# rezashkv/diffusion_pruning

Measured on NVIDIA B200. Metric: mixed_expert_unet_samples_steps_per_s, higher is better.
Workload: dtype bf16

## Files before the change

diffusion_pruning_b200/csrc/gemm_sm100.cu:

```cuda
#include "common.cuh"
#include "../../include/aptp_sm100.h"

namespace aptp {

constexpr int BM = 128;
constexpr int BK = 64;
constexpr int A_STAGE_BYTES = BM * BK * 2;
constexpr int EPI_PER_QUAD = 3;
constexpr int EPI_WARPS = 4 * EPI_PER_QUAD;
constexpr int GEMM_THREADS = 128 + EPI_WARPS * 32;
#define GEMM_CTRL_REGS "56"
#define GEMM_EPI_REGS "152"
constexpr int TMEM_COLS = 512;
constexpr int STG_WARP_BYTES = 32 * 64;
constexpr int STG_BYTES = EPI_WARPS * STG_WARP_BYTES;
constexpr int MAX_SMEM_SEGS = 96;
constexpr int SSEG_BYTES = MAX_SMEM_SEGS * 48;
constexpr int TILE_CACHE = 160;
constexpr int STILE_BYTES = TILE_CACHE * 16;
constexpr int SBIAS_BYTES = EPI_WARPS * 128 * 4;

struct GemmParams {
  CUtensorMap tmap_a;
  CUtensorMap tmap_b;
  CUtensorMap tmap_out;
  int out_tma;
  const aptp_gemm_seg* segs;
  const aptp_gemm_tile* tiles;
  int n_tiles;
  int n_segs;
  int a_mode;
  int batch, Ho, Wo;
  int bn, bw, bh, bb;
  int lbw, lbh;
  int stages;
  int k_tap_pitch;
  void* out;
  int out_ld, out_mode;
  const float* bias;
  const float* rowvec;
  int rowvec_ld, rows_per_sample;
  const void* residual;
  int res_ld;
  const float* gate;
  int gate_ld, gate_group;
  const float* border_tab;
  int tab_ld;
  int flags;
  const float* ln_colsum;
  const float2* ln_rowstats;
  float2* rowstat_out;
  int rowstat_chunks;
  float* gn_sum;
  float* gn_sq;
  int gn_ld, gn_blocks;
  int a_stat;
  int halo;
  CUtensorMap tmap_a2;
  CUtensorMap tmap_b2;
// ... 73 lines not shown
    v[q * 4 + 2] += f.z;
    v[q * 4 + 3] += f.w;
  }
}

__device__ __forceinline__ void ln_bias_apply32(float* v, const float* bias, const float* cs, float mu, float rstd) {
  const uint64_t r2 = pack_f32x2(rstd, rstd);
  const float nm = -mu * rstd;
  const uint64_t n2 = pack_f32x2(nm, nm);
#pragma unroll
  for (int q = 0; q < 8; ++q) {
    const float4 b = *(reinterpret_cast<const float4*>(bias) + q);
    const float4 c = *(reinterpret_cast<const float4*>(cs) + q);
    uint64_t a0 = fma_f32x2(r2, pack_f32x2(v[q * 4 + 0], v[q * 4 + 1]), pack_f32x2(b.x, b.y));
    uint64_t a1 = fma_f32x2(r2, pack_f32x2(v[q * 4 + 2], v[q * 4 + 3]), pack_f32x2(b.z, b.w));
    a0 = fma_f32x2(n2, pack_f32x2(c.x, c.y), a0);
    a1 = fma_f32x2(n2, pack_f32x2(c.z, c.w), a1);
    unpack_f32x2(a0, v[q * 4 + 0], v[q * 4 + 1]);
    unpack_f32x2(a1, v[q * 4 + 2], v[q * 4 + 3]);
  }
}

enum { EPI_BF16 = 0, EPI_GEGLU = 1, EPI_F32 = 2, EPI_NCHW = 3 };
#ifdef APTP_GEMM_TRACE
__device__ long long g_gemm_trace[512][16];
#define TRACE_T0() const long long _t0 = clock64(); long long _tw[2] = {0, 0}
#define TRACE_ADD(slot) if (lane == 0) { g_gemm_trace[blockIdx.x][slot] += clock64() - _t0; g_gemm_trace[blockIdx.x][slot + 1] += _tw[1]; if (slot == 2) g_gemm_trace[blockIdx.x][4] += _tw[0]; }
#define TRACE_WAIT(slot, expr) [&]() { const long long _w0 = clock64(); const bool _r = (expr); _tw[slot & 1] += clock64() - _w0; return _r; }()
#else
#define TRACE_T0()
#define TRACE_ADD(slot)
#define TRACE_WAIT(slot, expr) (expr)
#endif
template <int kEpi, bool k2Sm>
__global__ void __cluster_dims__(2, 1, 1) __launch_bounds__(GEMM_THREADS, 1)
grouped_gemm_kernel(const __grid_constant__ GemmParams p) {
  constexpr bool kGeglu = (kEpi == EPI_GEGLU);
  extern __shared__ uint8_t smem_raw[];
  uint8_t* smem = reinterpret_cast<uint8_t*>((reinterpret_cast<uintptr_t>(smem_raw) + 1023) & ~uintptr_t(1023));
  const int stages = p.stages;
  const uint32_t stage_bytes = ((p.a_stat || p.halo) ? 0u : (uint32_t)A_STAGE_BYTES) + (uint32_t)p.bn * (k2Sm ? 64u : 128u);
  const uint32_t ring_off = p.halo ? (uint32_t)p.halo * HALO_BYTES : (uint32_t)p.a_stat * A_STAGE_BYTES;
  uint8_t* stg_base = smem + ring_off + (size_t)stages * stage_bytes;
  float* sbias = reinterpret_cast<float*>(stg_base + STG_BYTES);
  aptp_gemm_seg* ssegs = reinterpret_cast<aptp_gemm_seg*>(stg_base + STG_BYTES + SBIAS_BYTES);
  aptp_gemm_tile* stiles = reinterpret_cast<aptp_gemm_tile*>(stg_base + STG_BYTES + SBIAS_BYTES + SSEG_BYTES);
  uint64_t* full_bar = reinterpret_cast<uint64_t*>(stg_base + STG_BYTES + SBIAS_BYTES + SSEG_BYTES + STILE_BYTES);
  uint64_t* empty_bar = full_bar + stages;
  uint64_t* tfull_bar = empty_bar + stages;
  uint64_t* tempty_bar = tfull_bar + 2;
  uint64_t* afull_bar = tempty_bar + 2;
  uint64_t* aempty_bar = afull_bar + A_STAT_MAX_CHUNKS;
  uint32_t* tmem_slot = reinterpret_cast<uint32_t*>(aempty_bar + A_STAT_MAX_CHUNKS);

  const int warp = __shfl_sync(0xffffffffu, (int)(threadIdx.x >> 5), 0);
  const int lane = threadIdx.x & 31;
#ifdef APTP_GEMM_TRACE
  const long long _t0_epi = clock64();
#endif
#define GEMM_ROLE_PROLOGUE()                                                                        \
  const uint32_t cta_rank = cluster_ctarank();                                                      \
  const int pair0 = blockIdx.x >> 1, pair_stride = gridDim.x >> 1, n_pairs = p.n_tiles >> 1;        \
  const aptp_gemm_seg* segs = (p.n_segs <= MAX_SMEM_SEGS) ? ssegs : p.segs;                         \
  const uint32_t tmem_base = *tmem_slot;                                                            \
  (void)cta_rank; (void)pair0; (void)pair_stride; (void)n_pairs; (void)segs; (void)tmem_base;

  if (warp == 0 && lane == 0) {
    tma_prefetch_desc(&p.tmap_a);
    tma_prefetch_desc(&p.tmap_b);
    if (p.out_tma) tma_prefetch_desc(&p.tmap_out);
    if (p.k2_chunks) {
      tma_prefetch_desc(&p.tmap_a2);
      tma_prefetch_desc(&p.tmap_b2);
    }
  }
  if (warp == 1) {
    if (lane == 0) {
      for (int s = 0; s < stages; ++s) {
        mbar_init(&full_bar[s], 1);
        mbar_init(&empty_bar[s], k2Sm ? 1 : 2);
      }
      for (int a = 0; a < 2; ++a) {
        mbar_init(&tfull_bar[a], 1);
        mbar_init(&tempty_bar[a], k2Sm ? 2 * EPI_WARPS : EPI_WARPS);
      }
      for (int a = 0; a < A_STAT_MAX_CHUNKS; ++a) {
        mbar_init(&afull_bar[a], 1);
        mbar_init(&aempty_bar[a], 1);
      }
      fence_barrier_init();
    }
    __syncwarp();
    if constexpr (k2Sm) {
      tmem_alloc_2sm(tmem_slot, TMEM_COLS);
      tmem_relinquish_2sm();
    } else {
      tmem_alloc(tmem_slot, TMEM_COLS);
      tmem_relinquish();
    }
  }
  const bool segs_in_smem = p.n_segs <= MAX_SMEM_SEGS;
  if (segs_in_smem) {
    const int4* src = reinterpret_cast<const int4*>(p.segs);
    int4* dst = reinterpret_cast<int4*>(ssegs);
    for (int i = threadIdx.x; i < p.n_segs * 3; i += blockDim.x) dst[i] = __ldg(src + i);
  }
  {
    const int pair0_ = blockIdx.x >> 1, pair_stride_ = gridDim.x >> 1, n_pairs_ = p.n_tiles >> 1;
    const uint32_t rank_ = cluster_ctarank();
    const int4* src = reinterpret_cast<const int4*>(p.tiles);
    int4* dst = reinterpret_cast<int4*>(stiles);
    for (int i = threadIdx.x; i < TILE_CACHE; i += blockDim.x) {
      const int pr = pair0_ + i * pair_stride_;
      if (pr < n_pairs_) dst[i] = __ldg(src + 2 * pr + rank_);
    }
  }
  tc_fence_before();
  cluster_sync_all();
  tc_fence_after();
  pdl_launch();
  pdl_wait();

// ... 295 lines not shown
            for (int k = 0; k < BK / 16; ++k) {
              if constexpr (k2Sm)
                umma_bf16_ss_2sm(d_tmem, da + (uint64_t)(k * 2), db + (uint64_t)(k * 2), idesc, (kb | k) != 0 ? 1u : 0u);
              else
                umma_bf16_ss(d_tmem, da + (uint64_t)(k * 2), db + (uint64_t)(k * 2), idesc, (kb | k) != 0 ? 1u : 0u);
            }
            if constexpr (k2Sm) umma_commit_2sm(&empty_bar[stage], (uint16_t)0x3);
            else umma_commit_mc(&empty_bar[stage], (uint16_t)0x3);
          }
          __syncwarp();
          advance(stage, phase, stages);
        }
        if (!ok) break;
        if (elect_one()) {
          if constexpr (k2Sm) umma_commit_2sm(&tfull_bar[acc], (uint16_t)0x3);
          else umma_commit(&tfull_bar[acc]);
        }
        __syncwarp();
        acc ^= 1;
        if (acc == 0) acc_phase ^= 1;
      }
      TRACE_ADD(2);
    }
  }
  } else {
    asm volatile("setmaxnreg.inc.sync.aligned.u32 " GEMM_EPI_REGS ";");
    GEMM_ROLE_PROLOGUE();
    const int ew = warp - 4;
    const int quad = warp & 3;
    const int cpar = ew >> 2;
    float* wbias = sbias + ew * 128;
    uint32_t chunk_rot = 0;
    const int r_own = quad * 32 + lane;
    uint8_t* stg = stg_base + ew * STG_WARP_BYTES;
    const uint32_t stg_own = smem_u32(stg) + lane * 64;
    const int own_sw = (lane >> 1) & 3;
    const int co_q = lane & 3;
    int acc = 0;
    uint32_t acc_phase = 0;
    constexpr bool geglu = kGeglu;
    constexpr bool bf16_out = (kEpi == EPI_BF16 || kEpi == EPI_GEGLU);
    int ti = 0;
    bool st_pending = false;
#ifdef APTP_GEMM_TRACE
    long long _tr_ld = 0, _tr_math = 0, _tr_st = 0, _tr_tfull = 0, _tr_busy = 0, _tr_tiles = 0;
#endif
    for (int pr = pair0; pr < n_pairs; pr += pair_stride, ++ti) {
      const aptp_gemm_tile tile = (ti < TILE_CACHE) ? stiles[ti] : p.tiles[2 * pr + cta_rank];
      if (tile.flags & APTP_TILE_SKIP) continue;
      const aptp_gemm_seg seg = segs[tile.seg];
      const bool placeholder = (tile.flags & APTP_TILE_PLACEHOLDER) != 0;
      TileGeom g;
      g.linear = (p.a_mode == APTP_A_LINEAR);
      g.m_base = tile.m_base;
      g.img0 = g.oy0 = g.ox0 = 0;
      if (!g.linear) {
        const int hw = p.Ho * p.Wo;
        g.img0 = tile.m_base / hw;
        const int rem = tile.m_base - g.img0 * hw;
        g.oy0 = rem / p.Wo;
        g.ox0 = rem - g.oy0 * p.Wo;
      }
      bool valid;
      int oy, ox;
      const int row = map_row(p, g, r_own, valid, oy, ox);
      valid = valid && !placeholder && (row < seg.row_end) && (row >= seg.row_begin);
      const int sample = valid ? row / p.rows_per_sample : 0;
      const int ycls = g.linear ? 1 : ((oy == 0) ? 0 : ((oy == p.Ho - 1) ? 2 : 1));
      const int xcls = g.linear ? 1 : ((ox == 0) ? 0 : ((ox == p.Wo - 1) ? 2 : 1));
      const float* tabp =
          (!kGeglu && p.border_tab) ? p.border_tab + seg.tab_off + (size_t)(ycls * 3 + xcls) * p.tab_ld : nullptr;
      int co_row[4];
      bool co_ok[4];
#pragma unroll
      for (int it = 0; it < 4; ++it) {
        int a, b;
        bool v;
        const int rr = map_row(p, g, quad * 32 + it * 8 + (lane >> 2), v, a, b);
        co_ok[it] = v && !placeholder && (rr < seg.row_end) && (rr >= seg.row_begin);
        co_row[it] = rr;
      }
      const int ocol_base = geglu ? tile.n0 / 2 : tile.n0;
      const int row0_q = tile.m_base + quad * 32;
      const bool rows_full = bf16_out && p.out_tma && !placeholder && row0_q >= seg.row_begin && row0_q + 32 <= seg.row_end;
      long long gn_row = -1;
      if ((kEpi == EPI_F32 || kEpi == EPI_BF16) && p.gn_sum != nullptr && !placeholder) {
        const int smp = tile.m_base / p.rows_per_sample;
        const int rem = tile.m_base - smp * p.rows_per_sample;
        int t_in_s;
        if (g.linear) {
          t_in_s = rem >> 7;
        } else {
          const int oy0 = rem / p.Wo, ox0 = rem - oy0 * p.Wo;
          t_in_s = (oy0 >> p.lbh) * (p.Wo >> p.lbw) + (ox0 >> p.lbw);
        }
        gn_row = ((long long)smp * p.gn_blocks + t_in_s * 4 + quad) * p.gn_ld;
      }

      uint4 rres[kEpi == EPI_BF16 ? 4 : 1];
      const bool use_res = (kEpi == EPI_BF16) && (p.residual != nullptr);
      auto load_res = [&](int col0) {
        if constexpr (kEpi == EPI_BF16) {
#pragma unroll
          for (int it = 0; it < 4; ++it) {
            rres[it] = make_uint4(0u, 0u, 0u, 0u);
            if (co_ok[it] && col0 + co_q * 8 < seg.n_valid)
              rres[it] = *reinterpret_cast<const uint4*>(reinterpret_cast<const __nv_bfloat16*>(p.residual) +
                                                         (size_t)co_row[it] * p.res_ld + seg.out_col_off + col0 +
                                                         co_q * 8);
          }
        }
      };
      constexpr bool f32_rows = (kEpi == EPI_F32);
      const bool use_res32 = f32_rows && (p.residual != nullptr) && (p.flags & APTP_EPI_RES_F32) != 0;
      uint4 rres32[f32_rows ? 2 : 1][f32_rows ? 4 : 1];
      auto load_res32 = [&](int col0) {
        if constexpr (f32_rows) {
#pragma unroll
          for (int h = 0; h < 2; ++h)
#pragma unroll
            for (int it = 0; it < 4; ++it) {
              rres32[h][it] = make_uint4(0u, 0u, 0u, 0u);
              if (co_ok[it] && col0 + h * 16 + co_q * 4 < seg.n_valid)
                rres32[h][it] = *reinterpret_cast<const uint4*>(reinterpret_cast<const float*>(p.residual) +
                                                                (size_t)co_row[it] * p.res_ld + seg.out_col_off + col0 +
                                                                h * 16 + co_q * 4);
            }
        }
      };
      const int w32_tile = (tile.flags >> 8) & 0xFF;
      const int out_cols_per_tile = geglu ? p.bn / 2 : (w32_tile ? w32_tile * 32 : p.bn);
      const int n_chunks = (out_cols_per_tile + 31) >> 5;
      const int c_first = (cpar + EPI_PER_QUAD - (int)(chunk_rot % EPI_PER_QUAD)) % EPI_PER_QUAD;
      chunk_rot += (uint32_t)n_chunks;
      const bool ln_fold = (p.flags & APTP_EPI_LN_FOLD) != 0;
      float bias_h = 0.f, bias_g = 0.f, cs_h = 0.f, cs_g = 0.f;
      auto load_bias = [&](int c) {
        const int col0 = ocol_base + c * 32;
        bias_h = bias_g = cs_h = cs_g = 0.f;
        if (p.bias && col0 + lane < seg.n_valid) {
          if (geglu) {
            bias_h = __ldg(p.bias + seg.vec_off + tile.n0 + c * 32 + lane);
            bias_g = __ldg(p.bias + seg.vec_off + tile.n0 + p.bn / 2 + c * 32 + lane);
          } else {
            bias_h = __ldg(p.bias + seg.vec_off + col0 + lane);
          }
        }
        if (ln_fold && col0 + lane < seg.n_valid) {
          if (geglu) {
            cs_h = __ldg(p.ln_colsum + seg.vec_off + tile.n0 + c * 32 + lane);
            cs_g = __ldg(p.ln_colsum + seg.vec_off + tile.n0 + p.bn / 2 + c * 32 + lane);
          } else {
            cs_h = __ldg(p.ln_colsum + seg.vec_off + col0 + lane);
          }
        }
      };
      float ln_mu = 0.f, ln_rstd = 1.f;
      if (ln_fold && valid) {
        const float2 ms = __ldg(p.ln_rowstats + row);
        ln_mu = ms.x;
        ln_rstd = ms.y;
      }
      if (c_first < n_chunks) {
        if (use_res && ocol_base + c_first * 32 < seg.n_store) load_res(ocol_base + c_first * 32);
        if (use_res32 && ocol_base + c_first * 32 < seg.n_store) load_res32(ocol_base + c_first * 32);
        load_bias(c_first);
      }

#ifdef APTP_GEMM_TRACE
      const long long _e0 = clock64();
      const bool got = mbar_wait(&tfull_bar[acc], acc_phase, p.abort_flag);
      const long long _e1 = clock64();
      _tr_tfull += _e1 - _e0;
#else
      const bool got = mbar_wait(&tfull_bar[acc], acc_phase, p.abort_flag);
#endif
      if (!got) break;
      tc_fence_after();
      asm volatile("" : "+f"(ln_mu), "+f"(ln_rstd));
      bool released = false;
      auto release_acc = [&]() {
        tc_fence_before();
        __syncwarp();
        if (lane == 0) {
          if constexpr (k2Sm) mbar_arrive_rank(&tempty_bar[acc], 0u);
          else mbar_arrive(&tempty_bar[acc]);
        }
      };
      const uint32_t t_addr = tmem_base + ((uint32_t)(quad * 32) << 16) + (uint32_t)(acc * p.bn);

#ifdef APTP_DBG_NOEPI
      if (p.n_tiles < 0)
#endif
      for (int c = c_first; c < n_chunks; c += EPI_PER_QUAD) {
        const int col0 = ocol_base + c * 32;
        if (col0 >= seg.n_store) break;
        const int n_ok = seg.n_valid - col0;
        if (st_pending) {
// ... 76 lines not shown
            release_acc();
            released = true;
          }
#endif
#pragma unroll
          for (int j = 0; j < 32; ++j) v[j] = __uint_as_float(ra[j]);
          if (ln_fold) ln_bias_apply32(v, wbias, wbias + 64, ln_mu, ln_rstd);
          else if (p.bias) add32_smem(v, wbias);
          if (p.bias || ln_fold) {
            __syncwarp();
            if (more) load_bias(c + EPI_PER_QUAD);
          }
          if (p.rowvec && valid) add32(v, p.rowvec + (size_t)sample * p.rowvec_ld + col0, n_ok);
          if (tabp) add32(v, tabp + col0, n_ok);
          if (p.gate && valid) {
            const float* gp = p.gate + (size_t)sample * p.gate_ld;
#pragma unroll
            for (int j = 0; j < 32; ++j)
              if (j < n_ok) v[j] *= __ldg(gp + (col0 + j) / p.gate_group);
          }
          if (p.flags & APTP_EPI_SILU) {
#pragma unroll
            for (int j = 0; j < 32; ++j) v[j] = silu_f(v[j]);
          }
        }

#ifdef APTP_GEMM_TRACE
        const long long _c2 = clock64();
        _tr_math += _c2 - _c1;
#endif
        if constexpr (bf16_out) {
          uint4* stg4 = reinterpret_cast<uint4*>(stg);
          if (kEpi == EPI_BF16 && use_res) {
#pragma unroll
            for (int it = 0; it < 4; ++it) {
              const int rl = it * 8 + (lane >> 2);
              stg4[rl * 4 + (co_q ^ ((rl >> 1) & 3))] = rres[it];
            }
            __syncwarp();
            uint4 w4[4];
#pragma unroll
            for (int q = 0; q < 4; ++q) w4[q] = stg4[lane * 4 + (q ^ own_sw)];
#pragma unroll
            for (int q = 0; q < 4; ++q) {
              v[q * 8 + 0] += bf16_lo(w4[q].x);
              v[q * 8 + 1] += bf16_hi(w4[q].x);
              v[q * 8 + 2] += bf16_lo(w4[q].y);
              v[q * 8 + 3] += bf16_hi(w4[q].y);
              v[q * 8 + 4] += bf16_lo(w4[q].z);
              v[q * 8 + 5] += bf16_hi(w4[q].z);
              v[q * 8 + 6] += bf16_lo(w4[q].w);
              v[q * 8 + 7] += bf16_hi(w4[q].w);
            }
            __syncwarp();
            if (more) load_res(col0 + 32 * EPI_PER_QUAD);
          }
          if (n_ok < 32) {
#pragma unroll
            for (int j = 0; j < 32; ++j)
              if (j >= n_ok) v[j] = 0.f;
          }
          if (kEpi == EPI_BF16 && p.rowstat_out && valid) {
            uint64_t su2 = pack_f32x2(0.f, 0.f), sq2 = su2;
#pragma unroll
            for (int j = 0; j < 32; j += 2) {
              const uint64_t x2 = pack_f32x2(v[j], v[j + 1]);
              su2 = add_f32x2(su2, x2);
              sq2 = fma_f32x2(x2, x2, sq2);
            }
            float s0, s1, q0, q1;
            unpack_f32x2(su2, s0, s1);
            unpack_f32x2(sq2, q0, q1);
            p.rowstat_out[(size_t)row * p.rowstat_chunks + ((seg.out_col_off + col0) >> 5)] =
                make_float2(s0 + s1, q0 + q1);
          }
#ifdef APTP_DBG_NOSTAGE
          if (v[0] == 1.2345e30f) p.abort_flag[1] = 1;
          if (p.n_tiles >= 0) continue;
#endif
#pragma unroll
          for (int q = 0; q < 4; ++q)
            stg4[lane * 4 + (q ^ own_sw)] =
                make_uint4(pack_bf16(v[q * 8 + 0], v[q * 8 + 1]), pack_bf16(v[q * 8 + 2], v[q * 8 + 3]),
                           pack_bf16(v[q * 8 + 4], v[q * 8 + 5]), pack_bf16(v[q * 8 + 6], v[q * 8 + 7]));
          if (rows_full && col0 + 32 <= seg.n_store) {
            fence_proxy_async();
            __syncwarp();
            if (lane == 0) {
              tma_store_2d(&p.tmap_out, stg, seg.out_col_off + col0, row0_q);
              bulk_commit();
            }
            st_pending = true;
            continue;
          }
          __syncwarp();
          __nv_bfloat16* obase = reinterpret_cast<__nv_bfloat16*>(p.out) + seg.out_col_off + col0 + co_q * 8;
          const bool col_ok = col0 + co_q * 8 < seg.n_store;
          uint4 o4[4];
#pragma unroll
          for (int it = 0; it < 4; ++it) {
            const int rl = it * 8 + (lane >> 2);
            o4[it] = stg4[rl * 4 + (co_q ^ ((rl >> 1) & 3))];
          }
#ifdef APTP_DBG_NOSTORE
          if (o4[0].x == 0x12345678u && o4[1].y == 0x9abcdef0u && o4[2].z == 0x0fedcba9u && o4[3].w == 0x87654321u)
#endif
#pragma unroll
          for (int it = 0; it < 4; ++it)
            if (co_ok[it] && col_ok) *reinterpret_cast<uint4*>(obase + (size_t)co_row[it] * p.out_ld) = o4[it];
          if constexpr (kEpi == EPI_BF16) {
            if (gn_row >= 0) {
              float cs[8], cq[8];
#pragma unroll
              for (int e = 0; e < 8; ++e) cs[e] = cq[e] = 0.f;
#pragma unroll
              for (int it = 0; it < 4; ++it) {
                if (co_ok[it]) {
                  const uint32_t wds[4] = {o4[it].x, o4[it].y, o4[it].z, o4[it].w};
#pragma unroll
                  for (int e = 0; e < 4; ++e) {
                    const float f0 = bf16_lo(wds[e]), f1 = bf16_hi(wds[e]);
                    cs[2 * e] += f0;
                    cs[2 * e + 1] += f1;
                    cq[2 * e] = fmaf(f0, f0, cq[2 * e]);
                    cq[2 * e + 1] = fmaf(f1, f1, cq[2 * e + 1]);
                  }
                }
              }
#pragma unroll
              for (int o = 4; o < 32; o <<= 1) {
#pragma unroll
                for (int e = 0; e < 8; ++e) {
                  cs[e] += __shfl_xor_sync(0xffffffffu, cs[e], o);
                  cq[e] += __shfl_xor_sync(0xffffffffu, cq[e], o);
                }
              }
              if (lane < 4 && col_ok) {
                const long long gi = gn_row + seg.out_col_off + col0 + co_q * 8;
                *reinterpret_cast<float4*>(p.gn_sum + gi) = make_float4(cs[0], cs[1], cs[2], cs[3]);
                *reinterpret_cast<float4*>(p.gn_sum + gi + 4) = make_float4(cs[4], cs[5], cs[6], cs[7]);
                *reinterpret_cast<float4*>(p.gn_sq + gi) = make_float4(cq[0], cq[1], cq[2], cq[3]);
                *reinterpret_cast<float4*>(p.gn_sq + gi + 4) = make_float4(cq[4], cq[5], cq[6], cq[7]);
              }
            }
          }
          __syncwarp();
        } else if constexpr (f32_rows) {
          uint4* stg4 = reinterpret_cast<uint4*>(stg);
          if (n_ok < 32) {
#pragma unroll
            for (int j = 0; j < 32; ++j)
              if (j >= n_ok) v[j] = 0.f;
          }
#pragma unroll
          for (int h = 0; h < 2; ++h) {
#pragma unroll
            for (int q = 0; q < 4; ++q)
              stg4[lane * 4 + (q ^ own_sw)] =
                  make_uint4(__float_as_uint(v[h * 16 + q * 4 + 0]), __float_as_uint(v[h * 16 + q * 4 + 1]),
                             __float_as_uint(v[h * 16 + q * 4 + 2]), __float_as_uint(v[h * 16 + q * 4 + 3]));
            __syncwarp();
            float* obase = reinterpret_cast<float*>(p.out) + seg.out_col_off + col0 + h * 16 + co_q * 4;
            const bool col_ok = col0 + h * 16 + co_q * 4 < seg.n_store;
            uint4 o4[4];
#pragma unroll
            for (int it = 0; it < 4; ++it) {
              const int rl = it * 8 + (lane >> 2);
              o4[it] = stg4[rl * 4 + (co_q ^ ((rl >> 1) & 3))];
            }
            if (use_res32) {
#pragma unroll
              for (int it = 0; it < 4; ++it) {
                o4[it].x = __float_as_uint(__uint_as_float(o4[it].x) + __uint_as_float(rres32[h][it].x));
                o4[it].y = __float_as_uint(__uint_as_float(o4[it].y) + __uint_as_float(rres32[h][it].y));
                o4[it].z = __float_as_uint(__uint_as_float(o4[it].z) + __uint_as_float(rres32[h][it].z));
                o4[it].w = __float_as_uint(__uint_as_float(o4[it].w) + __uint_as_float(rres32[h][it].w));
              }
            }
#pragma unroll
            for (int it = 0; it < 4; ++it)
              if (co_ok[it] && col_ok) *reinterpret_cast<uint4*>(obase + (size_t)co_row[it] * p.out_ld) = o4[it];
            if (gn_row >= 0) {
              float cs[4] = {0.f, 0.f, 0.f, 0.f}, cq[4] = {0.f, 0.f, 0.f, 0.f};
#pragma unroll
              for (int it = 0; it < 4; ++it) {
                if (co_ok[it]) {
                  const float f0 = __uint_as_float(o4[it].x), f1 = __uint_as_float(o4[it].y);
                  const float f2 = __uint_as_float(o4[it].z), f3 = __uint_as_float(o4[it].w);
                  cs[0] += f0; cs[1] += f1; cs[2] += f2; cs[3] += f3;
                  cq[0] = fmaf(f0, f0, cq[0]); cq[1] = fmaf(f1, f1, cq[1]);
                  cq[2] = fmaf(f2, f2, cq[2]); cq[3] = fmaf(f3, f3, cq[3]);
                }
              }
#pragma unroll
              for (int o = 4; o < 32; o <<= 1) {
#pragma unroll
                for (int e = 0; e < 4; ++e) {
                  cs[e] += __shfl_xor_sync(0xffffffffu, cs[e], o);
                  cq[e] += __shfl_xor_sync(0xffffffffu, cq[e], o);
                }
              }
              if (lane < 4 && col_ok) {
                const long long gi = gn_row + seg.out_col_off + col0 + h * 16 + co_q * 4;
                *reinterpret_cast<float4*>(p.gn_sum + gi) = make_float4(cs[0], cs[1], cs[2], cs[3]);
                *reinterpret_cast<float4*>(p.gn_sq + gi) = make_float4(cq[0], cq[1], cq[2], cq[3]);
              }
            }
            __syncwarp();
          }
          if (use_res32 && more) load_res32(col0 + 32 * EPI_PER_QUAD);
        } else if (valid) {
          if (n_ok < 32) {
#pragma unroll
            for (int j = 0; j < 32; ++j)
              if (j >= n_ok) v[j] = 0.f;
          }
          {
            float* op = reinterpret_cast<float*>(p.out);
            const int pix = row - sample * p.rows_per_sample;
#pragma unroll
            for (int j = 0; j < 32; ++j)
              if (j < n_ok) op[((size_t)sample * p.out_ld + col0 + j) * p.rows_per_sample + pix] = v[j];
          }
        }
#ifdef APTP_GEMM_TRACE
        _tr_st += clock64() - _c2;
#endif
      }
      if (!released) release_acc();
#ifdef APTP_GEMM_TRACE
      _tr_busy += clock64() - _e1;
      _tr_tiles += 1;
#endif
      acc ^= 1;
      if (acc == 0) acc_phase ^= 1;
    }
    if (lane == 0) bulk_wait0();
#ifdef APTP_GEMM_TRACE
    if (lane == 0 && ew < 2) {
      g_gemm_trace[blockIdx.x][6 + 3 * ew] += _tr_tfull;
      g_gemm_trace[blockIdx.x][7 + 3 * ew] += _tr_busy;
      g_gemm_trace[blockIdx.x][8 + 3 * ew] += _tr_tiles;
      if (ew == 0) {
// ... 11 lines not shown
  tc_fence_before();
  cluster_sync_all();
  if (warp == 1) {
    tc_fence_after();
    if constexpr (k2Sm) tmem_dealloc_2sm(*tmem_slot, TMEM_COLS);
    else tmem_dealloc(*tmem_slot, TMEM_COLS);
  }
}

#ifdef APTP_GEMM_TRACE
}
extern "C" int aptp_debug_gemm_trace(long long* host_out, int reset) {
  if (host_out && cudaMemcpyFromSymbol(host_out, aptp::g_gemm_trace, sizeof(long long) * 512 * 16) != cudaSuccess) return -1;
  if (reset) {
    static long long zeros[512 * 16];
    if (cudaMemcpyToSymbol(aptp::g_gemm_trace, zeros, sizeof(zeros)) != cudaSuccess) return -1;
  }
  return 0;
}
namespace aptp {
#endif
static int g_gemm_smem_set = 0;
static int g_gemm_max_clusters = 0;
static int g_gemm_2sm = 1;
static int g_gemm_2sm_mink = 1280;
static int g_conv_halo = 1;

}

using namespace aptp;

static int gemm_max_clusters() {
  if (!g_gemm_smem_set) {
    const void* fns[8] = {(const void*)grouped_gemm_kernel<EPI_BF16, false>, (const void*)grouped_gemm_kernel<EPI_GEGLU, false>,
                          (const void*)grouped_gemm_kernel<EPI_F32, false>,  (const void*)grouped_gemm_kernel<EPI_NCHW, false>,
                          (const void*)grouped_gemm_kernel<EPI_BF16, true>,  (const void*)grouped_gemm_kernel<EPI_GEGLU, true>,
                          (const void*)grouped_gemm_kernel<EPI_F32, true>,   (const void*)grouped_gemm_kernel<EPI_NCHW, true>};
    for (int i = 0; i < 8; ++i)
      if (cudaFuncSetAttribute(fns[i], cudaFuncAttributeMaxDynamicSharedMemorySize, 227 * 1024) != cudaSuccess) return 0;
    const char* e = getenv("APTP_GEMM_1SM");
    g_gemm_2sm = !(e && e[0] == '1');
    const char* hl = getenv("APTP_CONV_HALO");
    if (hl && hl[0] == '0') g_conv_halo = 0;
    const char* mk = getenv("APTP_GEMM_2SM_MINK");
    if (mk && atoi(mk) > 0) g_gemm_2sm_mink = atoi(mk);
    g_gemm_smem_set = 1;
  }
  if (!g_gemm_max_clusters) {
    cudaLaunchConfig_t cfg;
    memset(&cfg, 0, sizeof(cfg));
    cfg.gridDim = dim3(sm_count() & ~1, 1, 1);
    cfg.blockDim = dim3(GEMM_THREADS, 1, 1);
    cfg.dynamicSmemBytes = 227 * 1024;
    cudaLaunchAttribute attr;
    attr.id = cudaLaunchAttributeClusterDimension;
    attr.val.clusterDim.x = 2;
    attr.val.clusterDim.y = 1;
    attr.val.clusterDim.z = 1;
    cfg.attrs = &attr;
    cfg.numAttrs = 1;
    int n = 0;
    if (cudaOccupancyMaxActiveClusters(&n, grouped_gemm_kernel<EPI_BF16, true>, &cfg) != cudaSuccess || n <= 0) return 0;
    g_gemm_max_clusters = n;
  }
  return g_gemm_max_clusters;
}

extern "C" int aptp_gemm_max_pairs(void) { return gemm_max_clusters(); }

extern "C" int aptp_grouped_gemm_fwd(const aptp_gemm_args* a, void* stream_) {
  cudaStream_t stream = reinterpret_cast<cudaStream_t>(stream_);
  APTP_REQUIRE(a != nullptr, "aptp_grouped_gemm_fwd: null args");
  APTP_REQUIRE(a->a && a->w && a->out && a->segs && a->tiles, "aptp_grouped_gemm_fwd: null pointer");
  if (a->n_tiles == 0) return APTP_OK;
  APTP_REQUIRE(a->n_tiles % 2 == 0, "aptp_grouped_gemm_fwd: tiles must come in pairs (n_tiles=%d is odd)", a->n_tiles);
  APTP_REQUIRE(a->bn >= 32 && a->bn <= 256 && a->bn % 32 == 0, "aptp_grouped_gemm_fwd: bn=%d must be a multiple of 32 in [32,256]", a->bn);
  APTP_REQUIRE(a->a_ld % 8 == 0 && a->w_ld % 8 == 0, "aptp_grouped_gemm_fwd: a_ld/w_ld must be multiples of 8 (16-byte rows)");
  APTP_REQUIRE(a->out_mode == APTP_OUT_F32_NCHW || a->out_ld % 8 == 0, "aptp_grouped_gemm_fwd: out_ld must be a multiple of 8");
  APTP_REQUIRE((reinterpret_cast<uintptr_t>(a->a) & 15) == 0 && (reinterpret_cast<uintptr_t>(a->w) & 15) == 0 &&
                   (reinterpret_cast<uintptr_t>(a->out) & 15) == 0,
               "aptp_grouped_gemm_fwd: operands must be 16-byte aligned");
  APTP_REQUIRE(a->rows_per_sample > 0, "aptp_grouped_gemm_fwd: rows_per_sample must be > 0");
  if (a->flags & APTP_EPI_RES_F32)
    APTP_REQUIRE(a->residual != nullptr && a->out_mode == APTP_OUT_F32 && a->res_ld % 4 == 0 &&
                     (reinterpret_cast<uintptr_t>(a->residual) & 15) == 0,
                 "aptp_grouped_gemm_fwd: APTP_EPI_RES_F32 needs an fp32 residual (16-byte aligned rows) and APTP_OUT_F32");
  else
    APTP_REQUIRE(a->residual == nullptr || (a->out_mode == APTP_OUT_BF16 && a->res_ld % 8 == 0),
                 "aptp_grouped_gemm_fwd: a bf16 residual needs a bf16 output and res_ld %% 8 == 0");
  APTP_REQUIRE(a->a_rows < (1ll << 31), "aptp_grouped_gemm_fwd: too many rows");
  if (a->flags & APTP_EPI_GN_STATS) {
    APTP_REQUIRE(a->gn_stats && a->gn_stats_sq && (a->out_mode == APTP_OUT_F32 || a->out_mode == APTP_OUT_BF16) &&
                     !(a->flags & APTP_EPI_GEGLU),
                 "aptp_grouped_gemm_fwd: APTP_EPI_GN_STATS needs both partial planes and a row output (fp32 or bf16)");
    APTP_REQUIRE(a->rows_per_sample % 128 == 0 && a->gn_blocks == a->rows_per_sample / 32 && a->gn_ld % 4 == 0,
// ... 79 lines not shown
    uint64_t strides[3] = {(uint64_t)a->a2_ld * 2, (uint64_t)a->W * a->a2_ld * 2, (uint64_t)a->H * a->W * a->a2_ld * 2};
    uint32_t box[4] = {BK, 8, 16, 1};
    int rc = make_tmap_bf16(&p.tmap_a2, a->a2, 4, dims, strides, box);
    if (rc) return rc;
    uint64_t wdims[2] = {(uint64_t)a->w2_ld, (uint64_t)a->w2_rows};
    uint64_t wstrides[1] = {(uint64_t)a->w2_ld * 2};
    uint32_t wbox[2] = {BK, (uint32_t)a->bn / 2};
    rc = make_tmap_bf16(&p.tmap_b2, a->w2, 2, wdims, wstrides, wbox);
    if (rc) return rc;
    p.k2_chunks = (a->a2_k + BK - 1) / BK;
  }
  p.segs = a->segs;
  p.tiles = a->tiles;
  p.n_tiles = a->n_tiles;
  p.n_segs = a->n_segs;
  p.a_mode = a->a_mode;
  p.batch = a->batch;
  p.Ho = Ho;
  p.Wo = Wo;
  p.bn = a->bn;
  p.bw = a->a_mode == APTP_A_LINEAR ? BM : a->bw;
  p.bh = a->a_mode == APTP_A_LINEAR ? 1 : a->bh;
  p.bb = a->a_mode == APTP_A_LINEAR ? 1 : a->bb;
  APTP_REQUIRE((p.bw & (p.bw - 1)) == 0 && (p.bh & (p.bh - 1)) == 0, "aptp_grouped_gemm_fwd: box extents must be powers of two");
  p.lbw = 0;
  while ((1 << p.lbw) < p.bw) ++p.lbw;
  p.lbh = 0;
  while ((1 << p.lbh) < p.bh) ++p.lbh;
  p.k_tap_pitch = a->k_tap_pitch;
  p.out = a->out;
  p.out_ld = a->out_ld;
  p.out_mode = a->out_mode;
  p.out_tma = 0;
  {
    static int tma_store = -1;
    if (tma_store < 0) {
      const char* e = getenv("APTP_GEMM_TMA_STORE");
      tma_store = !(e && e[0] == '0');
    }
    if (tma_store && a->a_mode == APTP_A_LINEAR && a->out_mode == APTP_OUT_BF16 && !(a->flags & APTP_EPI_GN_STATS) &&
        (reinterpret_cast<uintptr_t>(a->out) & 15) == 0) {
      const uint64_t out_cols = (uint64_t)a->out_ld;
      int rc = make_tmap_store64(&p.tmap_out, a->out, false, out_cols, (uint64_t)a->a_rows, (uint64_t)a->out_ld * 2);
      if (rc) return rc;
      p.out_tma = 1;
    }
  }
  p.bias = a->bias;
  p.rowvec = a->rowvec;
  p.rowvec_ld = a->rowvec_ld;
  p.rows_per_sample = a->rows_per_sample;
  p.residual = a->residual;
  p.res_ld = a->res_ld;
  p.gate = a->gate;
  p.gate_ld = a->gate_ld;
  p.gate_group = a->gate_group > 0 ? a->gate_group : 1;
  p.border_tab = a->border_tab;
  p.tab_ld = a->tab_ld;
  p.flags = a->flags;
  p.ln_colsum = a->ln_colsum;
  p.ln_rowstats = reinterpret_cast<const float2*>(a->ln_rowstats);
  p.rowstat_out = reinterpret_cast<float2*>(a->rowstat_out);
  p.rowstat_chunks = a->rowstat_chunks;
  const bool gn = (a->flags & APTP_EPI_GN_STATS) != 0;
  p.gn_sum = gn ? a->gn_stats : nullptr;
  p.gn_sq = gn ? a->gn_stats_sq : nullptr;
  p.gn_ld = a->gn_ld;
  p.gn_blocks = a->gn_blocks;
  p.abort_flag = device_abort_flag();
  APTP_REQUIRE(p.abort_flag != nullptr, "aptp_grouped_gemm_fwd: could not allocate abort flag");

  p.a_stat = 0;
  if (a->a_stat_chunks > 0) {
    APTP_REQUIRE(a->a_mode == APTP_A_LINEAR && a->a_stat_chunks <= A_STAT_MAX_CHUNKS,
                 "aptp_grouped_gemm_fwd: A-stationary mode needs a linear layer with at most %d K chunks", A_STAT_MAX_CHUNKS);
    p.a_stat = a->a_stat_chunks;
  }
  const int stage_bytes = ((p.a_stat || halo) ? 0 : A_STAGE_BYTES) + a->bn * (two_sm ? 64 : 128);
  p.halo = 0;
  if (halo) {
    p.halo = 2;
    const int b8 = 8 * stage_bytes;
    if (225 * 1024 - 1024 - 512 - STG_BYTES - SBIAS_BYTES - SSEG_BYTES - STILE_BYTES - 3 * HALO_BYTES >= b8) p.halo = 3;
  }
  const int a_region = p.halo ? p.halo * HALO_BYTES : p.a_stat * A_STAGE_BYTES;
  const int budget = 225 * 1024 - 1024  - 512  - STG_BYTES  - SBIAS_BYTES -
                     SSEG_BYTES - STILE_BYTES - a_region;
  int stages = budget / stage_bytes;
  if (stages > 8) stages = 8;
  APTP_REQUIRE(stages >= 2, "aptp_grouped_gemm_fwd: tile too large for shared memory");
  p.stages = stages;
  const size_t smem_bytes = (size_t)a_region + (size_t)stages * stage_bytes + STG_BYTES + SBIAS_BYTES +
                            SSEG_BYTES + STILE_BYTES + 1024 + 512;
  const int n_pairs = a->n_tiles / 2;
  int grid = 2 * (n_pairs < g_gemm_max_clusters ? n_pairs : g_gemm_max_clusters);
  if (p.a_stat) {
    APTP_REQUIRE(a->a_stat_pairs > 0 && a->a_stat_pairs <= g_gemm_max_clusters && n_pairs % a->a_stat_pairs == 0,
                 "aptp_grouped_gemm_fwd: A-stationary tile list needs 0 < a_stat_pairs <= %d dividing the pair count", g_gemm_max_clusters);
    grid = 2 * a->a_stat_pairs;
  }
#define APTP_LAUNCH_GEMM(EPI)                                                                  \
  do {                                                                                         \
    if (two_sm) APTP_CUDA_CHECK(launch_pdl(grouped_gemm_kernel<EPI, true>, dim3(grid), dim3(GEMM_THREADS), smem_bytes, stream, p)); \
    else APTP_CUDA_CHECK(launch_pdl(grouped_gemm_kernel<EPI, false>, dim3(grid), dim3(GEMM_THREADS), smem_bytes, stream, p));       \
  } while (0)
  if (a->flags & APTP_EPI_GEGLU) APTP_LAUNCH_GEMM(EPI_GEGLU);
  else if (a->out_mode == APTP_OUT_BF16) APTP_LAUNCH_GEMM(EPI_BF16);
  else if (a->out_mode == APTP_OUT_F32) APTP_LAUNCH_GEMM(EPI_F32);
  else APTP_LAUNCH_GEMM(EPI_NCHW);
#undef APTP_LAUNCH_GEMM
  APTP_CUDA_CHECK(cudaGetLastError());
  return APTP_OK;
}
```

Baseline: 1365.

## Load GEMM epilogue residuals via TMA and extend TMA bulk stores to f32/GN outputs

Adds a TMA tensor map for the residual input. Each epilogue warp prefetches its residual tile into a dedicated shared-memory slot, tracked by a per-warp mbarrier, instead of loading it through registers and staging it. TMA bulk stores are extended to f32 outputs that carry a residual, and to outputs that also accumulate GroupNorm stats. The extra residual and f32 staging buffers consume shared memory that previously went to pipeline stages, which can reduce the stage count. More template variants are instantiated.

```diff
diff --git a/diffusion_pruning_b200/csrc/gemm_sm100.cu b/diffusion_pruning_b200/csrc/gemm_sm100.cu
--- a/diffusion_pruning_b200/csrc/gemm_sm100.cu
+++ b/diffusion_pruning_b200/csrc/gemm_sm100.cu
@@ -14,6 +14,7 @@
 constexpr int TMEM_COLS = 512;
 constexpr int STG_WARP_BYTES = 32 * 64;
 constexpr int STG_BYTES = EPI_WARPS * STG_WARP_BYTES;
+constexpr int STG_F32_BYTES = 2 * STG_BYTES;
 constexpr int MAX_SMEM_SEGS = 96;
 constexpr int SSEG_BYTES = MAX_SMEM_SEGS * 48;
 constexpr int TILE_CACHE = 160;
@@ -25,6 +26,8 @@
   CUtensorMap tmap_b;
   CUtensorMap tmap_out;
   int out_tma;
+  CUtensorMap tmap_res;
+  int res_tma;
   const aptp_gemm_seg* segs;
   const aptp_gemm_tile* tiles;
   int n_tiles;
@@ -164,7 +167,7 @@
 #define TRACE_ADD(slot)
 #define TRACE_WAIT(slot, expr) (expr)
 #endif
-template <int kEpi, bool k2Sm>
+template <int kEpi, bool k2Sm, bool kResTma>
 __global__ void __cluster_dims__(2, 1, 1) __launch_bounds__(GEMM_THREADS, 1)
 grouped_gemm_kernel(const __grid_constant__ GemmParams p) {
   constexpr bool kGeglu = (kEpi == EPI_GEGLU);
@@ -173,17 +176,22 @@
   const int stages = p.stages;
   const uint32_t stage_bytes = ((p.a_stat || p.halo) ? 0u : (uint32_t)A_STAGE_BYTES) + (uint32_t)p.bn * (k2Sm ? 64u : 128u);
   const uint32_t ring_off = p.halo ? (uint32_t)p.halo * HALO_BYTES : (uint32_t)p.a_stat * A_STAGE_BYTES;
-  uint8_t* stg_base = smem + ring_off + (size_t)stages * stage_bytes;
-  float* sbias = reinterpret_cast<float*>(stg_base + STG_BYTES);
-  aptp_gemm_seg* ssegs = reinterpret_cast<aptp_gemm_seg*>(stg_base + STG_BYTES + SBIAS_BYTES);
-  aptp_gemm_tile* stiles = reinterpret_cast<aptp_gemm_tile*>(stg_base + STG_BYTES + SBIAS_BYTES + SSEG_BYTES);
-  uint64_t* full_bar = reinterpret_cast<uint64_t*>(stg_base + STG_BYTES + SBIAS_BYTES + SSEG_BYTES + STILE_BYTES);
+  constexpr uint32_t RES_SLOT_BYTES = (kEpi == EPI_F32) ? 2 * STG_WARP_BYTES : STG_WARP_BYTES;
+  uint8_t* res_base = smem + ring_off + (size_t)stages * stage_bytes;
+  uint8_t* stg_base = res_base + (kResTma ? EPI_WARPS * RES_SLOT_BYTES : 0u);
+  const uint32_t stg_warp_bytes = (kEpi == EPI_F32 && kResTma) ? 2 * STG_WARP_BYTES : STG_WARP_BYTES;
+  uint8_t* stg_end = stg_base + EPI_WARPS * stg_warp_bytes;
+  float* sbias = reinterpret_cast<float*>(stg_end);
+  aptp_gemm_seg* ssegs = reinterpret_cast<aptp_gemm_seg*>(stg_end + SBIAS_BYTES);
+  aptp_gemm_tile* stiles = reinterpret_cast<aptp_gemm_tile*>(stg_end + SBIAS_BYTES + SSEG_BYTES);
+  uint64_t* full_bar = reinterpret_cast<uint64_t*>(stg_end + SBIAS_BYTES + SSEG_BYTES + STILE_BYTES);
   uint64_t* empty_bar = full_bar + stages;
   uint64_t* tfull_bar = empty_bar + stages;
   uint64_t* tempty_bar = tfull_bar + 2;
   uint64_t* afull_bar = tempty_bar + 2;
   uint64_t* aempty_bar = afull_bar + A_STAT_MAX_CHUNKS;
-  uint32_t* tmem_slot = reinterpret_cast<uint32_t*>(aempty_bar + A_STAT_MAX_CHUNKS);
+  uint64_t* res_bar = aempty_bar + A_STAT_MAX_CHUNKS;
+  uint32_t* tmem_slot = reinterpret_cast<uint32_t*>(res_bar + EPI_WARPS);
 
   const int warp = __shfl_sync(0xffffffffu, (int)(threadIdx.x >> 5), 0);
   const int lane = threadIdx.x & 31;
@@ -201,6 +209,7 @@
     tma_prefetch_desc(&p.tmap_a);
     tma_prefetch_desc(&p.tmap_b);
     if (p.out_tma) tma_prefetch_desc(&p.tmap_out);
+    if (kResTma) tma_prefetch_desc(&p.tmap_res);
     if (p.k2_chunks) {
       tma_prefetch_desc(&p.tmap_a2);
       tma_prefetch_desc(&p.tmap_b2);
@@ -220,6 +229,7 @@
         mbar_init(&afull_bar[a], 1);
         mbar_init(&aempty_bar[a], 1);
       }
+      for (int w = 0; w < EPI_WARPS; ++w) mbar_init(&res_bar[w], 1);
       fence_barrier_init();
     }
     __syncwarp();
@@ -581,7 +591,9 @@
     float* wbias = sbias + ew * 128;
     uint32_t chunk_rot = 0;
     const int r_own = quad * 32 + lane;
-    uint8_t* stg = stg_base + ew * STG_WARP_BYTES;
+    uint8_t* stg = stg_base + ew * stg_warp_bytes;
+    uint8_t* rslot = res_base + ew * RES_SLOT_BYTES;
+    uint32_t res_phase = 0;
     const uint32_t stg_own = smem_u32(stg) + lane * 64;
     const int own_sw = (lane >> 1) & 3;
     const int co_q = lane & 3;
@@ -631,7 +643,7 @@
       }
       const int ocol_base = geglu ? tile.n0 / 2 : tile.n0;
       const int row0_q = tile.m_base + quad * 32;
-      const bool rows_full = bf16_out && p.out_tma && !placeholder && row0_q >= seg.row_begin && row0_q + 32 <= seg.row_end;
+      const bool rows_full = p.out_tma && !placeholder && row0_q >= seg.row_begin && row0_q + 32 <= seg.row_end;
       long long gn_row = -1;
       if ((kEpi == EPI_F32 || kEpi == EPI_BF16) && p.gn_sum != nullptr && !placeholder) {
         const int smp = tile.m_base / p.rows_per_sample;
@@ -646,6 +658,20 @@
         gn_row = ((long long)smp * p.gn_blocks + t_in_s * 4 + quad) * p.gn_ld;
       }
 
+#ifndef APTP_DBG_NOEPI
+      constexpr bool res_tma = kResTma;
+#else
+      constexpr bool res_tma = false;
+#endif
+      auto issue_res = [&](int col0) {
+        if (elect_one()) {
+          mbar_expect_tx(&res_bar[ew], RES_SLOT_BYTES);
+          tma_load_2d(rslot, &p.tmap_res, &res_bar[ew], seg.out_col_off + col0, row0_q);
+          if constexpr (kEpi == EPI_F32)
+            tma_load_2d(rslot + STG_WARP_BYTES, &p.tmap_res, &res_bar[ew], seg.out_col_off + col0 + 16, row0_q);
+        }
+        __syncwarp();
+      };
       uint4 rres[kEpi == EPI_BF16 ? 4 : 1];
       const bool use_res = (kEpi == EPI_BF16) && (p.residual != nullptr);
       auto load_res = [&](int col0) {
@@ -711,8 +737,11 @@
         ln_rstd = ms.y;
       }
       if (c_first < n_chunks) {
-        if (use_res && ocol_base + c_first * 32 < seg.n_store) load_res(ocol_base + c_first * 32);
-        if (use_res32 && ocol_base + c_first * 32 < seg.n_store) load_res32(ocol_base + c_first * 32);
+        if ((use_res || use_res32) && ocol_base + c_first * 32 < seg.n_store) {
+          if (res_tma) issue_res(ocol_base + c_first * 32);
+          else if (use_res) load_res(ocol_base + c_first * 32);
+          else load_res32(ocol_base + c_first * 32);
+        }
         load_bias(c_first);
       }
 
@@ -855,15 +884,23 @@
         if constexpr (bf16_out) {
           uint4* stg4 = reinterpret_cast<uint4*>(stg);
           if (kEpi == EPI_BF16 && use_res) {
-#pragma unroll
-            for (int it = 0; it < 4; ++it) {
-              const int rl = it * 8 + (lane >> 2);
-              stg4[rl * 4 + (co_q ^ ((rl >> 1) & 3))] = rres[it];
-            }
-            __syncwarp();
-            uint4 w4[4];
-#pragma unroll
-            for (int q = 0; q < 4; ++q) w4[q] = stg4[lane * 4 + (q ^ own_sw)];
+            uint4* w4 = rres;
+            if (res_tma) {
+              if (!mbar_wait(&res_bar[ew], res_phase, p.abort_flag)) break;
+              res_phase ^= 1;
+              const uint4* r4 = reinterpret_cast<const uint4*>(rslot);
+#pragma unroll
+              for (int q = 0; q < 4; ++q) w4[q] = r4[lane * 4 + (q ^ own_sw)];
+            } else {
+#pragma unroll
+              for (int it = 0; it < 4; ++it) {
+                const int rl = it * 8 + (lane >> 2);
+                stg4[rl * 4 + (co_q ^ ((rl >> 1) & 3))] = rres[it];
+              }
+              __syncwarp();
+#pragma unroll
+              for (int q = 0; q < 4; ++q) w4[q] = stg4[lane * 4 + (q ^ own_sw)];
+            }
 #pragma unroll
             for (int q = 0; q < 4; ++q) {
               v[q * 8 + 0] += bf16_lo(w4[q].x);
@@ -875,8 +912,14 @@
               v[q * 8 + 6] += bf16_lo(w4[q].w);
               v[q * 8 + 7] += bf16_hi(w4[q].w);
             }
-            __syncwarp();
-            if (more) load_res(col0 + 32 * EPI_PER_QUAD);
+            if (res_tma) {
+              fence_proxy_async();
+              __syncwarp();
+              if (more) issue_res(col0 + 32 * EPI_PER_QUAD);
+            } else {
+              __syncwarp();
+              if (more) load_res(col0 + 32 * EPI_PER_QUAD);
+            }
           }
           if (n_ok < 32) {
 #pragma unroll
@@ -906,7 +949,8 @@
             stg4[lane * 4 + (q ^ own_sw)] =
                 make_uint4(pack_bf16(v[q * 8 + 0], v[q * 8 + 1]), pack_bf16(v[q * 8 + 2], v[q * 8 + 3]),
                            pack_bf16(v[q * 8 + 4], v[q * 8 + 5]), pack_bf16(v[q * 8 + 6], v[q * 8 + 7]));
-          if (rows_full && col0 + 32 <= seg.n_store) {
+          const bool bulk = rows_full && col0 + 32 <= seg.n_store;
+          if (bulk) {
             fence_proxy_async();
             __syncwarp();
             if (lane == 0) {
@@ -914,9 +958,10 @@
               bulk_commit();
             }
             st_pending = true;
-            continue;
-          }
-          __syncwarp();
+            if (gn_row < 0) continue;
+          } else {
+            __syncwarp();
+          }
           __nv_bfloat16* obase = reinterpret_cast<__nv_bfloat16*>(p.out) + seg.out_col_off + col0 + co_q * 8;
           const bool col_ok = col0 + co_q * 8 < seg.n_store;
           uint4 o4[4];
@@ -928,9 +973,11 @@
 #ifdef APTP_DBG_NOSTORE
           if (o4[0].x == 0x12345678u && o4[1].y == 0x9abcdef0u && o4[2].z == 0x0fedcba9u && o4[3].w == 0x87654321u)
 #endif
-#pragma unroll
-          for (int it = 0; it < 4; ++it)
-            if (co_ok[it] && col_ok) *reinterpret_cast<uint4*>(obase + (size_t)co_row[it] * p.out_ld) = o4[it];
+          if (!bulk) {
+#pragma unroll
+            for (int it = 0; it < 4; ++it)
+              if (co_ok[it] && col_ok) *reinterpret_cast<uint4*>(obase + (size_t)co_row[it] * p.out_ld) = o4[it];
+          }
           if constexpr (kEpi == EPI_BF16) {
             if (gn_row >= 0) {
               float cs[8], cq[8];
@@ -969,20 +1016,53 @@
           }
           __syncwarp();
         } else if constexpr (f32_rows) {
-          uint4* stg4 = reinterpret_cast<uint4*>(stg);
+          if (use_res32 && res_tma) {
+            if (!mbar_wait(&res_bar[ew], res_phase, p.abort_flag)) break;
+            res_phase ^= 1;
+            const uint4* r4 = reinterpret_cast<const uint4*>(rslot);
+#pragma unroll
+            for (int h = 0; h < 2; ++h)
+#pragma unroll
+              for (int q = 0; q < 4; ++q) rres32[h][q] = r4[h * 128 + lane * 4 + (q ^ own_sw)];
+#pragma unroll
+            for (int h = 0; h < 2; ++h)
+#pragma unroll
+              for (int q = 0; q < 4; ++q) {
+                v[h * 16 + q * 4 + 0] += __uint_as_float(rres32[h][q].x);
+                v[h * 16 + q * 4 + 1] += __uint_as_float(rres32[h][q].y);
+                v[h * 16 + q * 4 + 2] += __uint_as_float(rres32[h][q].z);
+                v[h * 16 + q * 4 + 3] += __uint_as_float(rres32[h][q].w);
+              }
+            fence_proxy_async();
+            __syncwarp();
+            if (more) issue_res(col0 + 32 * EPI_PER_QUAD);
+          }
           if (n_ok < 32) {
 #pragma unroll
             for (int j = 0; j < 32; ++j)
               if (j >= n_ok) v[j] = 0.f;
           }
+          const bool bulk = kResTma && rows_full && col0 + 32 <= seg.n_store;
 #pragma unroll
           for (int h = 0; h < 2; ++h) {
+            uint4* stg4 = reinterpret_cast<uint4*>(stg) + (kResTma ? h * 128 : 0);
 #pragma unroll
             for (int q = 0; q < 4; ++q)
               stg4[lane * 4 + (q ^ own_sw)] =
                   make_uint4(__float_as_uint(v[h * 16 + q * 4 + 0]), __float_as_uint(v[h * 16 + q * 4 + 1]),
                              __float_as_uint(v[h * 16 + q * 4 + 2]), __float_as_uint(v[h * 16 + q * 4 + 3]));
-            __syncwarp();
+            if (bulk) {
+              fence_proxy_async();
+              __syncwarp();
+              if (lane == 0) {
+                tma_store_2d(&p.tmap_out, stg4, seg.out_col_off + col0 + h * 16, row0_q);
+                bulk_commit();
+              }
+              st_pending = true;
+              if (gn_row < 0) continue;
+            } else {
+              __syncwarp();
+            }
             float* obase = reinterpret_cast<float*>(p.out) + seg.out_col_off + col0 + h * 16 + co_q * 4;
             const bool col_ok = col0 + h * 16 + co_q * 4 < seg.n_store;
             uint4 o4[4];
@@ -991,7 +1071,7 @@
               const int rl = it * 8 + (lane >> 2);
               o4[it] = stg4[rl * 4 + (co_q ^ ((rl >> 1) & 3))];
             }
-            if (use_res32) {
+            if (use_res32 && !res_tma) {
 #pragma unroll
               for (int it = 0; it < 4; ++it) {
                 o4[it].x = __float_as_uint(__uint_as_float(o4[it].x) + __uint_as_float(rres32[h][it].x));
@@ -1000,9 +1080,11 @@
                 o4[it].w = __float_as_uint(__uint_as_float(o4[it].w) + __uint_as_float(rres32[h][it].w));
               }
             }
-#pragma unroll
-            for (int it = 0; it < 4; ++it)
-              if (co_ok[it] && col_ok) *reinterpret_cast<uint4*>(obase + (size_t)co_row[it] * p.out_ld) = o4[it];
+            if (!bulk) {
+#pragma unroll
+              for (int it = 0; it < 4; ++it)
+                if (co_ok[it] && col_ok) *reinterpret_cast<uint4*>(obase + (size_t)co_row[it] * p.out_ld) = o4[it];
+            }
             if (gn_row >= 0) {
               float cs[4] = {0.f, 0.f, 0.f, 0.f}, cq[4] = {0.f, 0.f, 0.f, 0.f};
 #pragma unroll
@@ -1031,7 +1113,7 @@
             }
             __syncwarp();
           }
-          if (use_res32 && more) load_res32(col0 + 32 * EPI_PER_QUAD);
+          if (use_res32 && !res_tma && more) load_res32(col0 + 32 * EPI_PER_QUAD);
         } else if (valid) {
           if (n_ok < 32) {
 #pragma unroll
@@ -1109,11 +1191,14 @@
 
 static int gemm_max_clusters() {
   if (!g_gemm_smem_set) {
-    const void* fns[8] = {(const void*)grouped_gemm_kernel<EPI_BF16, false>, (const void*)grouped_gemm_kernel<EPI_GEGLU, false>,
-                          (const void*)grouped_gemm_kernel<EPI_F32, false>,  (const void*)grouped_gemm_kernel<EPI_NCHW, false>,
-                          (const void*)grouped_gemm_kernel<EPI_BF16, true>,  (const void*)grouped_gemm_kernel<EPI_GEGLU, true>,
-                          (const void*)grouped_gemm_kernel<EPI_F32, true>,   (const void*)grouped_gemm_kernel<EPI_NCHW, true>};
-    for (int i = 0; i < 8; ++i)
+    const void* fns[12] = {
+        (const void*)grouped_gemm_kernel<EPI_BF16, false, false>, (const void*)grouped_gemm_kernel<EPI_GEGLU, false, false>,
+        (const void*)grouped_gemm_kernel<EPI_F32, false, false>,  (const void*)grouped_gemm_kernel<EPI_NCHW, false, false>,
+        (const void*)grouped_gemm_kernel<EPI_BF16, true, false>,  (const void*)grouped_gemm_kernel<EPI_GEGLU, true, false>,
+        (const void*)grouped_gemm_kernel<EPI_F32, true, false>,   (const void*)grouped_gemm_kernel<EPI_NCHW, true, false>,
+        (const void*)grouped_gemm_kernel<EPI_BF16, false, true>,  (const void*)grouped_gemm_kernel<EPI_F32, false, true>,
+        (const void*)grouped_gemm_kernel<EPI_BF16, true, true>,   (const void*)grouped_gemm_kernel<EPI_F32, true, true>};
+    for (int i = 0; i < 12; ++i)
       if (cudaFuncSetAttribute(fns[i], cudaFuncAttributeMaxDynamicSharedMemorySize, 227 * 1024) != cudaSuccess) return 0;
     const char* e = getenv("APTP_GEMM_1SM");
     g_gemm_2sm = !(e && e[0] == '1');
@@ -1137,7 +1222,7 @@
     cfg.attrs = &attr;
     cfg.numAttrs = 1;
     int n = 0;
-    if (cudaOccupancyMaxActiveClusters(&n, grouped_gemm_kernel<EPI_BF16, true>, &cfg) != cudaSuccess || n <= 0) return 0;
+    if (cudaOccupancyMaxActiveClusters(&n, grouped_gemm_kernel<EPI_BF16, true, false>, &cfg) != cudaSuccess || n <= 0) return 0;
     g_gemm_max_clusters = n;
   }
   return g_gemm_max_clusters;
@@ -1283,18 +1368,26 @@
   p.out_ld = a->out_ld;
   p.out_mode = a->out_mode;
   p.out_tma = 0;
+  p.res_tma = 0;
   {
     static int tma_store = -1;
     if (tma_store < 0) {
       const char* e = getenv("APTP_GEMM_TMA_STORE");
       tma_store = !(e && e[0] == '0');
     }
-    if (tma_store && a->a_mode == APTP_A_LINEAR && a->out_mode == APTP_OUT_BF16 && !(a->flags & APTP_EPI_GN_STATS) &&
-        (reinterpret_cast<uintptr_t>(a->out) & 15) == 0) {
+    if (tma_store && a->a_mode == APTP_A_LINEAR &&
+        (a->out_mode == APTP_OUT_BF16 || (a->out_mode == APTP_OUT_F32 && a->residual != nullptr))) {
+      const bool f32 = a->out_mode == APTP_OUT_F32;
       const uint64_t out_cols = (uint64_t)a->out_ld;
-      int rc = make_tmap_store64(&p.tmap_out, a->out, false, out_cols, (uint64_t)a->a_rows, (uint64_t)a->out_ld * 2);
+      int rc = make_tmap_store64(&p.tmap_out, a->out, f32, out_cols, (uint64_t)a->a_rows, (uint64_t)a->out_ld * (f32 ? 4 : 2));
       if (rc) return rc;
       p.out_tma = 1;
+      if (a->residual) {
+        rc = make_tmap_store64(&p.tmap_res, a->residual, f32, (uint64_t)a->res_ld, (uint64_t)a->a_rows,
+                               (uint64_t)a->res_ld * (f32 ? 4 : 2));
+        if (rc) return rc;
+        p.res_tma = 1;
+      }
     }
   }
   p.bias = a->bias;
@@ -1328,20 +1421,23 @@
     p.a_stat = a->a_stat_chunks;
   }
   const int stage_bytes = ((p.a_stat || halo) ? 0 : A_STAGE_BYTES) + a->bn * (two_sm ? 64 : 128);
+  const bool f32_rows = a->out_mode == APTP_OUT_F32;
+  const int epi_bytes = ((f32_rows && p.res_tma) ? STG_F32_BYTES : STG_BYTES) +
+                        (p.res_tma ? (f32_rows ? STG_F32_BYTES : STG_BYTES) : 0);
   p.halo = 0;
   if (halo) {
     p.halo = 2;
     const int b8 = 8 * stage_bytes;
-    if (225 * 1024 - 1024 - 512 - STG_BYTES - SBIAS_BYTES - SSEG_BYTES - STILE_BYTES - 3 * HALO_BYTES >= b8) p.halo = 3;
+    if (225 * 1024 - 1024 - 512 - epi_bytes - SBIAS_BYTES - SSEG_BYTES - STILE_BYTES - 3 * HALO_BYTES >= b8) p.halo = 3;
   }
   const int a_region = p.halo ? p.halo * HALO_BYTES : p.a_stat * A_STAGE_BYTES;
-  const int budget = 225 * 1024 - 1024  - 512  - STG_BYTES  - SBIAS_BYTES -
+  const int budget = 225 * 1024 - 1024  - 512  - epi_bytes - SBIAS_BYTES -
                      SSEG_BYTES - STILE_BYTES - a_region;
   int stages = budget / stage_bytes;
   if (stages > 8) stages = 8;
   APTP_REQUIRE(stages >= 2, "aptp_grouped_gemm_fwd: tile too large for shared memory");
   p.stages = stages;
-  const size_t smem_bytes = (size_t)a_region + (size_t)stages * stage_bytes + STG_BYTES + SBIAS_BYTES +
+  const size_t smem_bytes = (size_t)a_region + (size_t)stages * stage_bytes + epi_bytes + SBIAS_BYTES +
                             SSEG_BYTES + STILE_BYTES + 1024 + 512;
   const int n_pairs = a->n_tiles / 2;
   int grid = 2 * (n_pairs < g_gemm_max_clusters ? n_pairs : g_gemm_max_clusters);
@@ -1350,15 +1446,17 @@
                  "aptp_grouped_gemm_fwd: A-stationary tile list needs 0 < a_stat_pairs <= %d dividing the pair count", g_gemm_max_clusters);
     grid = 2 * a->a_stat_pairs;
   }
-#define APTP_LAUNCH_GEMM(EPI)                                                                  \
+#define APTP_LAUNCH_GEMM(EPI, RT)                                                              \
   do {                                                                                         \
-    if (two_sm) APTP_CUDA_CHECK(launch_pdl(grouped_gemm_kernel<EPI, true>, dim3(grid), dim3(GEMM_THREADS), smem_bytes, stream, p)); \
-    else APTP_CUDA_CHECK(launch_pdl(grouped_gemm_kernel<EPI, false>, dim3(grid), dim3(GEMM_THREADS), smem_bytes, stream, p));       \
+    if (two_sm) APTP_CUDA_CHECK(launch_pdl(grouped_gemm_kernel<EPI, true, RT>, dim3(grid), dim3(GEMM_THREADS), smem_bytes, stream, p)); \
+    else APTP_CUDA_CHECK(launch_pdl(grouped_gemm_kernel<EPI, false, RT>, dim3(grid), dim3(GEMM_THREADS), smem_bytes, stream, p));       \
   } while (0)
-  if (a->flags & APTP_EPI_GEGLU) APTP_LAUNCH_GEMM(EPI_GEGLU);
-  else if (a->out_mode == APTP_OUT_BF16) APTP_LAUNCH_GEMM(EPI_BF16);
-  else if (a->out_mode == APTP_OUT_F32) APTP_LAUNCH_GEMM(EPI_F32);
-  else APTP_LAUNCH_GEMM(EPI_NCHW);
+  if (a->flags & APTP_EPI_GEGLU) APTP_LAUNCH_GEMM(EPI_GEGLU, false);
+  else if (a->out_mode == APTP_OUT_BF16 && p.res_tma) APTP_LAUNCH_GEMM(EPI_BF16, true);
+  else if (a->out_mode == APTP_OUT_BF16) APTP_LAUNCH_GEMM(EPI_BF16, false);
+  else if (a->out_mode == APTP_OUT_F32 && p.res_tma) APTP_LAUNCH_GEMM(EPI_F32, true);
+  else if (a->out_mode == APTP_OUT_F32) APTP_LAUNCH_GEMM(EPI_F32, false);
+  else APTP_LAUNCH_GEMM(EPI_NCHW, false);
 #undef APTP_LAUNCH_GEMM
   APTP_CUDA_CHECK(cudaGetLastError());
   return APTP_OK;
```

After: 1382, median of 6. 1.01x the previous value.
